# Happy-ZZX/PL-VIWO

Hardware: AMD Instinct MI355X
Metric: frames/sec (track+EKF update), 752x480 mono, 250 pts+80 lines; ATE vs CPU ref (higher is better)
Workload: dtype f64

## Files before the change

### pl-viwo_amd/csrc/camera_tracks.hpp

```cpp
#pragma once
#include <algorithm>
#include <cstdint>
#include <unordered_map>
#include <utility>
#include <vector>

#include "../../include/plviwo.h"

namespace plv {

inline int bounding_start_host(const plv_state_view &st, double t) {
  const int N = st.n_clones;
  if (N < 4) return -1;
  const double *ct = st.clone_time;
  if (t < ct[0] - st.dt_exp || t > ct[N - 1] + st.dt_exp) return -1;
  if (t > ct[N - 1]) return -1;
  int n_b = -1;
  for (int i = 0; i < N - 1; ++i)
    if (ct[i] - st.dt_exp <= t && t <= ct[i + 1] + st.dt_exp) {
      n_b = i;
      break;
    }
  if (n_b < 0) return -1;
  int start = n_b - 1;
  if (n_b - 1 < 0)
    start = 0;
  else if (n_b + 2 >= N)
    start = N - 4;
  if (start < 0 || start + 4 > N) return -1;
  return start;
}
inline bool has_bounding_poses(const plv_state_view &st, double t) { return bounding_start_host(st, t) >= 0; }

struct BoundingMemo {
  const plv_state_view &st;
  double t[40];
  int s0[40];
  int n = 0;
  explicit BoundingMemo(const plv_state_view &s) : st(s) {}
  int operator()(double tq) {
    for (int i = n - 1; i >= 0; --i)
      if (t[i] == tq) return s0[i];
    const int r = bounding_start_host(st, tq);
    if (n < 40) t[n] = tq, s0[n++] = r;
    return r;
  }
};

struct Track {
  static constexpr int W = 2;
  static constexpr int P = 3;
  std::vector<double> t;
  std::vector<float> uv, uvn;
  int li = -1;
  unsigned long long li_seq = 0;
};

struct LineTrack {
  static constexpr int W = 4;
  static constexpr int P = 6;
  std::vector<double> t;
  std::vector<float> uv, uvn;
  std::vector<int> points;
  int D = 0;
};

inline void copy_track_meta(Track &, const Track &) {}
inline void copy_track_meta(LineTrack &dst, const LineTrack &src) {
  if (dst.t.empty() && dst.points.empty()) {
    dst.D = src.D;
    dst.points = src.points;
  }
}

template <class TrackT> struct PoolCand {
  uint64_t id;
  TrackT tr;
};
template <class TrackT> using TrackMap = std::unordered_map<uint64_t, TrackT>;

template <class TrackT> void append_obs(TrackT &dst, const TrackT &src, size_t i) {
  constexpr size_t W = TrackT::W;
  dst.t.push_back(src.t[i]);
  dst.uv.insert(dst.uv.end(), src.uv.begin() + W * i, src.uv.begin() + W * (i + 1));
  dst.uvn.insert(dst.uvn.end(), src.uvn.begin() + W * i, src.uvn.begin() + W * (i + 1));
}

template <class TrackT> void give_back(TrackMap<TrackT> &unused, uint64_t id, const TrackT &src, size_t i) {
  TrackT &u = unused[id];
  copy_track_meta(u, src);
  append_obs(u, src, i);
}

template <class TrackT> void give_back_all(TrackMap<TrackT> &unused, PoolCand<TrackT> &c) {
  if (unused.find(c.id) == unused.end()) {
    unused.emplace(c.id, std::move(c.tr));
    c.tr = TrackT{};
    return;
  }
  for (size_t i = 0; i < c.tr.t.size(); ++i) give_back(unused, c.id, c.tr, i);
}

template <class TrackT, class Keep> size_t trim_track(TrackT &tr, Keep keep) {
  constexpr size_t W = TrackT::W;
  size_t n = 0;
  for (size_t i = 0; i < tr.t.size(); ++i) {
    if (!keep(i)) continue;
    if (n != i) {
      tr.t[n] = tr.t[i];
      std::copy(tr.uv.begin() + W * i, tr.uv.begin() + W * (i + 1), tr.uv.begin() + W * n);
      std::copy(tr.uvn.begin() + W * i, tr.uvn.begin() + W * (i + 1), tr.uvn.begin() + W * n);
    }
    ++n;
  }
  tr.t.resize(n);
  tr.uv.resize(W * n);
  tr.uvn.resize(W * n);
  return n;
}

template <class TrackT> size_t drop_before(TrackT &tr, double t) {
  return trim_track(tr, [&tr, t](size_t i) { return !(tr.t[i] < t); });
}

template <class TrackT> size_t trim_to_window(TrackMap<TrackT> &unused, uint64_t id, TrackT &tr, double dt, double t_new, double t_old) {
  return trim_track(tr, [&unused, id, &tr, dt, t_new, t_old](size_t i) {
    const double tm = tr.t[i] + dt;
    if (tm > t_new) {
      give_back(unused, id, tr, i);
      return false;
    }
    return !(tm < t_old);
  });
}

template <class TrackT> void take_pool(TrackMap<TrackT> &db, double t_old, double t_new, std::vector<PoolCand<TrackT>> &pool) {
  static thread_local std::vector<std::pair<uint64_t, typename TrackMap<TrackT>::iterator>> take;
  take.clear();
  for (auto it = db.begin(); it != db.end(); ++it) {
    bool older = false, newer = false;
    for (double t : it->second.t) {
      older = older || t < t_old;
      newer = newer || t > t_new;
    }
    if (older || !newer) take.emplace_back(it->first, it);
  }
  std::sort(take.begin(), take.end(), [](const auto &a, const auto &b) { return a.first < b.first; });
  pool.reserve(pool.size() + take.size());
  for (auto &tk : take) pool.push_back(PoolCand<TrackT>{tk.first, std::move(db.extract(tk.second).mapped())});
}

template <class TrackT> void sort_long_first(std::vector<PoolCand<TrackT>> &pool) {
  static thread_local std::vector<std::pair<int, int>> ord;
  ord.clear();
  for (size_t i = 0; i < pool.size(); ++i) ord.emplace_back(-(int)pool[i].tr.t.size(), (int)i);
  std::sort(ord.begin(), ord.end());
  std::vector<PoolCand<TrackT>> sorted;
  sorted.reserve(pool.size());
  for (const auto &o : ord) sorted.push_back(std::move(pool[(size_t)o.second]));
  pool.swap(sorted);
}

template <class TrackT>
void flatten_pool(const std::vector<PoolCand<TrackT>> &pool, std::vector<int> &ptr, std::vector<double> &t, std::vector<float> &uv, std::vector<float> &uvn) {
  constexpr size_t W = TrackT::W;
  ptr.assign(pool.size() + 1, 0);
  for (size_t f = 0; f < pool.size(); ++f) ptr[f + 1] = ptr[f] + (int)pool[f].tr.t.size();
  const size_t nobs = (size_t)ptr.back();
  t.resize(nobs), uv.resize(W * nobs), uvn.resize(W * nobs);
  for (size_t f = 0; f < pool.size(); ++f) {
    const TrackT &tr = pool[f].tr;
    std::copy(tr.t.begin(), tr.t.end(), t.begin() + ptr[f]);
    std::copy(tr.uv.begin(), tr.uv.end(), uv.begin() + W * ptr[f]);
    std::copy(tr.uvn.begin(), tr.uvn.end(), uvn.begin() + W * ptr[f]);
  }
}

struct CpiPoses {
  bool on = false, noise = false;
  std::vector<double> R, p, Q;
  std::vector<int> C;
};

template <class TrackT>
int cpi_attach(plv_ctx *ctx, const plv_state_view *st, const plv_cpi_table *cpi, bool noise, double dt, std::vector<PoolCand<TrackT>> &pool,
               TrackMap<TrackT> &unused, CpiPoses &out) {
  std::vector<double> tq;
  for (const PoolCand<TrackT> &c : pool)
    for (double t : c.tr.t) tq.push_back(t + dt);
  std::vector<double> Rq(9 * tq.size()), pq(3 * tq.size());
  std::vector<uint8_t> okq(tq.size());
// ... 94 lines not shown
      if (seen++ < S.n_skip[f] || fused_ran) continue;
      gather_obs(S.g, c.tr, i, cpi, ptr[f] + i);
    }
    S.sptr[q + 1] = (int)S.g.t.size();
    std::copy(feat_all + P * f, feat_all + P * (f + 1), S.feat.begin() + P * q);
    if (ids_out) ids_out[q] = c.id;
  }
}

template <class TrackT, class StartOf, class Whole>
int return_rejected(const std::vector<PoolCand<TrackT>> &pool, const Selection<TrackT> &S, double dt, StartOf &start_of, TrackMap<TrackT> &unused,
                    uint8_t *accepted_out, Whole whole) {
  int n_accepted = 0;
  for (size_t q = 0; q < S.sel.size(); ++q) {
    n_accepted += S.acc[q];
    if (accepted_out) accepted_out[q] = S.acc[q];
    if (S.acc[q] || whole(S.sel[q])) continue;
    const PoolCand<TrackT> &c = pool[S.sel[q]];
    for (size_t i = 0; i < c.tr.t.size(); ++i)
      if (start_of(c.tr.t[i] + dt) >= 0) give_back(unused, c.id, c.tr, i);
  }
  return n_accepted;
}

template <class TrackT> typename TrackMap<TrackT>::iterator put_track(TrackMap<TrackT> &db, uint64_t id, TrackT &tr) {
  auto ins = db.try_emplace(id);
  TrackT &d = ins.first->second;
  if (ins.second) {
    d = std::move(tr);
  } else {
    d.t.insert(d.t.end(), tr.t.begin(), tr.t.end());
    d.uv.insert(d.uv.end(), tr.uv.begin(), tr.uv.end());
    d.uvn.insert(d.uvn.end(), tr.uvn.begin(), tr.uvn.end());
  }
  return ins.first;
}

}
```

### pl-viwo_amd/csrc/jacobian_kernels.hip

```cpp
#include <hip/hip_runtime.h>
namespace plv {
#define JAC_NSTAMP 32
__device__ long long *g_jac_stamps = nullptr;
__device__ __forceinline__ void jac_stamp(int id) {
  long long *s = g_jac_stamps;
  if (s && threadIdx.x == 0) s[blockIdx.x * JAC_NSTAMP + id] = (long long)__builtin_amdgcn_s_memtime();
}
}
#define GATE_STAMP(id) jac_stamp(id)
#include "cam_models.hpp"
#include "gate_core.hpp"
#include "jacobian_kernels.hpp"
#include "nullspace_core.hpp"
#include "so3.hpp"

namespace plv {

__device__ int bounding_start(const JacParams &P, double t) {
  const int N = P.n_clones;
  if (N < 4) return -1;
  const double *ct = P.clone_time;
  if (t < ct[0] - P.dt_exp || t > ct[N - 1] + P.dt_exp) return -1;
  if (t > ct[N - 1]) return -1;
  int n_b = -1;
  for (int i = 0; i < N - 1; ++i)
    if (ct[i] - P.dt_exp <= t && t <= ct[i + 1] + P.dt_exp) {
      n_b = i;
      break;
    }
  if (n_b < 0) return -1;
  int start = n_b - 1;
  if (n_b - 1 < 0)
    start = 0;
  else if (n_b + 2 >= N)
    start = N - 4;
  if (start < 0 || start + 4 > N) return -1;
  return start;
}

struct Interp {
  M3 R;
  V3 p;
  M3 Ho[4];
  double lam[4];
  double dtj[6];
};
// ... 40 lines not shown
  const M3 Jl = Jl_so3(A_ori);
  M3 H0o = Rio;
  double lsum = 0;
#pragma unroll
  for (int w = 0; w < 3; ++w) {
    const M3 JinvW = inv3(Jl_so3(th[w]));
    H0o = ma(H0o, ms(mm(Jl, mm(JinvW, Rw[w])), -lam[w]));
    o.Ho[w + 1] = ms(mm(Jl, JinvW), lam[w]);
    o.lam[w + 1] = lam[w];
    lsum += lam[w];
  }
  o.Ho[0] = H0o;
  o.lam[0] = 1.0 - lsum;
  V3 dori{{0, 0, 0}}, dpos{{0, 0, 0}};
#pragma unroll
  for (int w = 0; w < 3; ++w) {
    dori = vadd(dori, vsc(th[w], lamd[w]));
    dpos = vadd(dpos, vsc(dp[w], lamd[w]));
  }
  const V3 top = vsc(mv(Jl, dori), -1.0);
#pragma unroll
  for (int i = 0; i < 3; ++i) {
    o.dtj[i] = top[i];
    o.dtj[3 + i] = dpos[i];
  }
}


struct WinTab {
  M3 R0, Rw[3], JinvW[3], Vi;
  V3 p0, th[3], dp[3];
  double vrow[3][3];
};
#define JAC_MAX_WIN 40

__device__ __forceinline__ void build_window_tables(const JacParams &P, WinTab *tab, const double *Rt = nullptr, const double *pt = nullptr) {
  const int nwin = max(P.n_clones - 3, 0);
  const int ntask = nwin * (Rt ? 3 : 2);
  const double *const R_est = P.clone_R, *const R_fej = P.clone_R_fej, *const p_est = P.clone_p, *const p_fej = P.clone_p_fej;
  for (int idx = threadIdx.x; idx < ntask * 3; idx += blockDim.x) {
    const int w = idx % 3, e = idx / 3;
    const bool second = e >= 2 * nwin;
    const int s0 = second ? e - 2 * nwin : e >> 1, fej = second ? 0 : e & 1;
    const double *Rs = second ? Rt : (fej ? R_fej : R_est), *ps = second ? pt : (fej ? p_fej : p_est);
    WinTab &T = tab[e];
    const M3 R0 = ldM(Rs + 9 * s0);
    const V3 p0 = ldV(ps + 3 * s0);
    const M3 Rw = mm(ldM(Rs + 9 * (s0 + 1 + w)), tp(R0));
    const V3 th = log_so3(Rw);
    T.Rw[w] = Rw;
    T.th[w] = th;
    T.dp[w] = vsub(ldV(ps + 3 * (s0 + 1 + w)), p0);
    const double d = P.clone_time[s0 + 1 + w] - P.clone_time[s0];
    T.vrow[w][0] = d;
    T.vrow[w][1] = d * d;
    T.vrow[w][2] = d * d * d;
    if (fej) T.JinvW[w] = inv3(Jl_so3(th));
    if (w == 0) {
      T.R0 = R0;
      T.p0 = p0;
    }
  }
  __syncthreads();
  for (int e = threadIdx.x; e < ntask; e += blockDim.x) {
    M3 V;
#pragma unroll
    for (int w = 0; w < 3; ++w)
// ... 1996 lines not shown
```

### pl-viwo_amd/csrc/line_api.hip

```cpp
#include <algorithm>
#include <chrono>
#include <cmath>
#include <cstring>
#include <atomic>
#include <condition_variable>
#include <functional>
#include <memory>
#include <map>
#include <mutex>
#include <thread>
#include <unordered_map>
#include <vector>

#include "line_host.hpp"
#include "cam_models.hpp"
#include "line_kernels.hpp"
#include "update_state.hpp"
#include "plv_internal.hpp"
#include "camera_tracks.hpp"
#include "update_tail.hpp"

using namespace plv;
using namespace plv::linehost;

// ... 37 lines not shown
  std::vector<float> uv, uvn;
  std::vector<uint8_t> has, flags;
  CpiPoses cpi;
  std::vector<double> lg_two_step;
  std::vector<uint8_t> ok_two_step;
  double us_pool = 0;
  plv_line_tracks view() const {
    plv_line_tracks all{};
    all.n_lines = Lp, all.obs_ptr = ptr.data(), all.obs_time = ot.data(), all.seg_uv = uv.data(), all.seg_uvn = uvn.data();
    all.D = D.data(), all.anchor_pt = anchor.data(), all.has_pt = has.data();
    if (cpi.on) all.res_R = cpi.R.data(), all.res_p = cpi.p.data();
    return all;
  }
};

struct LineTracker {
  LinePool pool_prep;
  LinesJob ujob;
  std::vector<float> lines_last;
  std::vector<uint64_t> ids_last;
  std::vector<int> rel_ptr_last{0};
  std::vector<uint64_t> rel_id_last;
  uint64_t currid = 1;
  bool walk_on_device = false;
  int walk_mode = 0;
  struct WalkInfo {
    int mode = 0, n_components = 0, longest_component = 0, n_chains = 0, fell_back = 0;
  } winfo;
  bool chains_valid = false;
  std::vector<FldChain> last_chains;
  int last_pts_extent = 0;
  DevBuf comps, recs, recs_sorted;
  bool prefetch = false;
  std::unordered_map<uint64_t, LineTrack> db;
  DevBuf half, map, work, pts, chains, counts, segs, seg_count, uv_in, uv_out;
  DevBuf lab, lab_cnt, lab_roots;
  hipStream_t ccl_stream = nullptr;
  hipEvent_t canny_done = nullptr, labels_ready = nullptr;
  PinBuf pin;
  hipEvent_t edges_ready = nullptr;
  std::vector<uint64_t> dec_ids;
  std::vector<double> dec_vals;
  const uint8_t *early_raw = nullptr;
  const unsigned *early_hist = nullptr;
  int early_w = 0, early_h = 0;
  int pending_which = -1, pending_fed = -1;
  bool defer_finish = false;
  std::function<void()> deferred;
  std::atomic<int> defer_state{0};
  struct TriState {
    bool valid = false;
    plv_state_view view;
    std::vector<double> clone_time, clone_R, clone_p;
    std::vector<int> clone_id;
  } tri_state;
  std::vector<float> cached;
  int cached_which = -1, cached_fed = -1;
  std::mutex mtx;
  linehost::Job job;
  std::thread worker;
  std::mutex jm;
  std::condition_variable jcv;
  std::atomic<int> job_state{0};
  struct FeedJob {
    plv_ctx *ctx = nullptr;
    double timestamp = 0, vps[6] = {0, 0, 0, 0, 0, 0};
    double K8[8] = {0, 0, 0, 0, 0, 0, 0, 0};
// ... 577 lines not shown
  auto F0 = std::chrono::steady_clock::now();
  const int nl = (int)lines.size() / 4;
  plv::counters().lines_detected += (unsigned long long)nl;
  std::vector<uint64_t> ids(nl);
  for (int i = 0; i < nl; ++i) ids[i] = ++T->currid;
  Assign A;
  assign_points_parallel(&T->host, fit_threads().load(std::memory_order_relaxed), lines.data(), nl, pts, pids, np, A);
  auto F1 = std::chrono::steady_clock::now();
  const int nk = (int)A.kept.size();
  std::vector<float> fl(4 * (size_t)nk);
  std::vector<uint64_t> fid(nk);
  for (int q = 0; q < nk; ++q) {
    std::copy(lines.begin() + 4 * A.kept[q], lines.begin() + 4 * A.kept[q] + 4, fl.begin() + 4 * q);
    fid[q] = ids[A.kept[q]];
  }
  const bool first = T->lines_last.empty();
  auto F_match = F1, F_und = F1;
  if (!first) {
    std::vector<int> match((size_t)std::max(nk, 1));
    match_lines_parallel(&T->host, fit_threads().load(std::memory_order_relaxed), fl.data(), nk, A.rel_ptr.data(), A.rel_id.data(), T->lines_last.data(),
                         (int)T->ids_last.size(), T->rel_ptr_last.data(), T->rel_id_last.data(), match.data());
    for (int q = 0; q < nk; ++q)
      if (match[q] >= 0) fid[q] = (uint64_t)(int)T->ids_last[match[q]];
    if (timing) F_match = std::chrono::steady_clock::now();
    std::vector<float> un(4 * (size_t)std::max(nk, 1));
    for (int q = 0; q < 2 * nk; ++q)
      undistort_model(cam_model, K8, fl[2 * (size_t)q], fl[2 * (size_t)q + 1], un[2 * (size_t)q], un[2 * (size_t)q + 1]);
    if (timing) F_und = std::chrono::steady_clock::now();
    for (int q = 0; q < nk; ++q) {
      const int D = plv_line_classification(fl.data() + 4 * q, vps);
      auto ins = T->db.try_emplace(fid[q]);
      const bool is_new = ins.second;
      LineTrack &tr = ins.first->second;
      if (is_new) {
        tr.D = D;
        tr.t.reserve(32);
        tr.uv.reserve(128);
        tr.uvn.reserve(128);
      }
      tr.t.push_back(timestamp);
      tr.uv.insert(tr.uv.end(), fl.begin() + 4 * q, fl.begin() + 4 * q + 4);
      tr.uvn.insert(tr.uvn.end(), un.begin() + 4 * q, un.begin() + 4 * q + 4);
      for (int p = A.rel_ptr[q]; p < A.rel_ptr[q + 1]; ++p) tr.points.push_back((int)A.rel_id[p]);
    }
  }
  T->lines_last.swap(fl);
  T->ids_last.swap(fid);
  T->rel_ptr_last = A.rel_ptr;
  T->rel_id_last = A.rel_id;
  if (timing) {
    auto us = [](auto a, auto b) { return std::chrono::duration<double, std::micro>(b - a).count(); };
    fprintf(stderr, "line feed: kept-line copy + match %.1f us, undistort %.1f us, classify + store -> end %.1f us\n", us(F1, F_match), us(F_match, F_und),
            us(F_und, std::chrono::steady_clock::now()));
    fprintf(stderr, "line feed: assignment %.1f us (%d lines x %d points), match + undistort + classify + store %.1f us (%d kept)\n", us(F0, F1), nl, np,
            us(F1, std::chrono::steady_clock::now()), nk);
  }
  return PLV_OK;
}

}
namespace plv {
int plv_line_tracker_feed_async_points(plv_ctx *ctx, double timestamp, const double *vps, int np, const float *pts, const uint64_t *pids) {
  if (!ctx || !vps || np < 0 || (np > 0 && (!pts || !pids))) return PLV_E_BADARG;
  LineTracker *T = ltr(ctx);
  std::lock_guard<std::mutex> lk(T->mtx);
  LineTracker::FeedJob &F = T->feed;
  F.pts.assign(pts, pts + 2 * (size_t)np);
  F.pids.assign(pids, pids + (size_t)np);
  const bool detecting = !T->walk_on_device && T->worker.joinable() && T->pending_which == PLV_PYR_CUR && T->pending_fed == plv_front_fed_count(ctx);
  if (!detecting) {
    F.pool_on = false;
    F.rc = feed_points_impl(ctx, T, timestamp, vps, np, F.pts.data(), F.pids.data(), ctx->cfg.intrinsics, ctx->cam_model);
    return F.rc;
  }
  g_feed_impl = feed_points_impl;
// ... 80 lines not shown
      if (seg_uvn) std::copy(tr.uvn.begin(), tr.uvn.end(), seg_uvn + 4 * (size_t)no);
      no += m;
      if (D) D[i] = tr.D;
      if (pts_ptr) {
        if (npt + (int)tr.points.size() > pts_cap) return PLV_E_CAPACITY;
        if (pt_ids) std::copy(tr.points.begin(), tr.points.end(), pt_ids + npt);
        npt += (int)tr.points.size();
      }
    } else if (D) {
      D[i] = 0;
    }
    obs_ptr[i + 1] = no;
    if (pts_ptr) pts_ptr[i + 1] = npt;
  }
  return PLV_OK;
}

int plv_line_db_remove(plv_ctx *ctx, const uint64_t *ids, int n_ids) {
  if (!ctx || (n_ids > 0 && !ids)) return PLV_E_BADARG;
  LineTracker *T = ltr(ctx);
  std::lock_guard<std::mutex> lk(T->mtx);
  for (int i = 0; i < n_ids; ++i) T->db.erase(ids[i]);
  return PLV_OK;
}

int plv_line_db_append_measurements(plv_ctx *ctx, uint64_t id, int n, const double *t, const float *seg_uv,
                                    const float *seg_uvn, int D, const int *point_ids, int n_pts) {
  if (!ctx || n < 0 || (n > 0 && (!t || !seg_uv || !seg_uvn)) || (n_pts > 0 && !point_ids)) return PLV_E_BADARG;
  LineTracker *T = ltr(ctx);
  std::lock_guard<std::mutex> lk(T->mtx);
  const bool is_new = T->db.find(id) == T->db.end();
  LineTrack &tr = T->db[id];
  if (is_new) tr.D = D;
  tr.t.insert(tr.t.end(), t, t + n);
  tr.uv.insert(tr.uv.end(), seg_uv, seg_uv + 4 * (size_t)n);
  tr.uvn.insert(tr.uvn.end(), seg_uvn, seg_uvn + 4 * (size_t)n);
  tr.points.insert(tr.points.end(), point_ids, point_ids + n_pts);
  return PLV_OK;
}

}
namespace plv {
void plv_line_defer_finish(plv_ctx *ctx, int on) { ltr(ctx, false)->defer_finish = on != 0; }
void plv_line_run_deferred(plv_ctx *ctx) { (void)ltr(ctx); }
}
extern "C" {

namespace {
struct LineWaitHook {
  plv_ctx *ctx;
  std::function<void()> *fn;
};
void line_wait_hook(void *arg) {
  LineWaitHook *h = (LineWaitHook *)arg;
  plv_tracker_run_deferred(h->ctx);
  if (h->fn && *h->fn) (*h->fn)();
}
}

namespace {
void form_line_pool(LineTracker *T, const PoolArgs &A, LinePool &R) {
  R = LinePool();
  R.valid = true;
  R.t_prev_frame = A.t_prev_frame, R.state_time = A.state_time, R.dt = A.dt, R.n_clones = A.n_clones;
  R.t_oldest = A.t_oldest, R.t_oldest2 = A.t_oldest2;
  const double dt = R.dt, t_oldest = R.t_oldest, t_oldest2 = R.t_oldest2;
  const PoolArgs *opt = &A;
  plv::HostPhase ph_scan("line pool: scan + take");
  {
    std::lock_guard<std::mutex> lk(T->mtx);
    R.db_size_before = (int)T->db.size();
    take_pool(T->db, t_oldest2 - dt, opt->t_prev_frame - dt, R.pool);
  }
  ph_scan.stop();
  plv::HostPhase ph_trim("line pool: trim + sort");
  R.n_pool = (int)R.pool.size();
  R.unused.reserve(R.pool.size());
  size_t kept_cands = 0;
  for (size_t ci = 0; ci < R.pool.size(); ++ci) {
    PoolCand<LineTrack> &c = R.pool[ci];
    if (trim_to_window(R.unused, c.id, c.tr, dt, opt->state_time + 0.01, t_oldest - 0.01) >= 2) {
      if (kept_cands != ci) R.pool[kept_cands] = std::move(c);
      ++kept_cands;
    }
  }
  R.pool.resize(kept_cands);
  sort_long_first(R.pool);
}
}

namespace {
void discard_line_pool(LineTracker *T) {
  LinePool &R = T->pool_prep;
  if (!R.valid) return;
  std::lock_guard<std::mutex> lk(T->mtx);
  auto put = [&](uint64_t id, LineTrack &tr) {
    const bool is_new = T->db.find(id) == T->db.end();
    LineTrack &d = T->db[id];
    if (is_new) {
      d = std::move(tr);
      return;
    }
    const size_t na = d.t.size(), nb = tr.t.size();
    std::vector<std::pair<double, std::pair<int, int>>> order;
    order.reserve(na + nb);
    for (size_t i = 0; i < na; ++i) order.push_back({d.t[i], {0, (int)i}});
    for (size_t i = 0; i < nb; ++i) order.push_back({tr.t[i], {1, (int)i}});
    std::stable_sort(order.begin(), order.end(), [](const auto &a, const auto &b) { return a.first < b.first; });
    LineTrack m;
    copy_track_meta(m, d);
    for (const auto &e : order) append_obs(m, e.second.first ? tr : d, (size_t)e.second.second);
    d = std::move(m);
  };
  for (auto &c : R.pool) put(c.id, c.tr);
  for (auto &kv : R.unused) put(kv.first, kv.second);
  R = LinePool();
}
}

}
namespace plv {
int plv_line_pool_prepare(plv_ctx *ctx, const plv_state_view *st, const plv_update_options *opt) {
  if (!ctx || !st || !opt || opt->cpi || st->n_clones < 2 || st->dt_state_id >= 0) return 1;
  LineTracker *T;
  {
    std::lock_guard<std::mutex> lk(g_mtx);
    auto it = g_lt.find(ctx);
    if (it == g_lt.end()) return 1;
    T = it->second;
  }
  {
    std::lock_guard<std::mutex> lk(T->jm);
    if (T->feed_state == 1) return 0;
  }
  T = ltr(ctx);
  if (T->feed.rc != PLV_OK) return 1;
  const PoolArgs A = PoolArgs::of(st, opt);
  const LinePool &R = T->pool_prep;
  if (R.valid && R.t_prev_frame == A.t_prev_frame && R.state_time == A.state_time && R.dt == A.dt && R.n_clones == A.n_clones && R.t_oldest == A.t_oldest &&
      R.t_oldest2 == A.t_oldest2)
    return 1;
  plv::HostPhase ph("update_lines: pool formed inside the point update's wait");
  discard_line_pool(T);
  form_line_pool(T, A, T->pool_prep);
  return 1;
// ... 369 lines not shown
```

### pl-viwo_amd/csrc/tracker_api.hip

```cpp
#include <algorithm>
#include <cmath>
#include <functional>
#include <memory>
#include <mutex>
#include <unordered_map>
#include <vector>

#include <sys/resource.h>
#include "plv_ctx.hpp"
#include "update_state.hpp"
#include "plv_internal.hpp"
#include "gate_stage.hpp"
#include "camera_tracks.hpp"
#include "update_tail.hpp"

using plv::Track;

namespace {

struct Tracker {
  std::vector<float> pts_last;
  std::vector<uint64_t> ids_last;
  std::vector<uint8_t> mask_last;
  uint64_t currid = 0;
  int detect_ahead = 2;
  bool ahead_deferred = false;
  bool defer_db = false;
  const plv_state_view *early_st = nullptr;
  const plv_update_options *early_lines = nullptr;
  int early_cap = 0;
  std::unordered_map<uint64_t, int> chain_index;
  bool chain_ok = false;
  std::function<void()> deferred_db;
  std::unordered_map<uint64_t, Track> db;
  struct UsedPoint {
    double p[3], newest;
  };
  std::unordered_map<uint64_t, UsedPoint> used;
  struct Listed {
    uint64_t id;
    Track tr;
    double p[3];
  };
  std::vector<Listed> last_slam, last_init;
  std::vector<uint64_t> dec_ids;
  std::vector<double> dec_vals;
  const plv_state_view *spec_st = nullptr;
  const plv_update_options *spec_opt = nullptr;
  std::function<void(int, const float *, const uint64_t *)> points_ready;
  unsigned long long feed_seq = 0;
  std::vector<double> frame_t;
  struct Spec {
    bool active = false;
    double t_prev_frame = 0, state_time = 0, dt = 0, t_oldest = 0, t_oldest2 = 0;
    int n_clones = 0, max_msckf = 0, max_obs = 0, k = 0, F = 0;
    std::unordered_map<uint64_t, int> index;
    std::vector<uint64_t> ids;
    std::vector<int> ptr, li, cols;
    std::vector<uint8_t> meta, prevalid, flags;
    std::vector<double> ot;
    std::vector<float> ouv, ouvn;
  } spec;
  std::mutex mtx;
};

std::mutex g_mtx;
std::unordered_map<plv_ctx *, Tracker *> g_trk;
// ... 284 lines not shown
    keep_mask();
    return PLV_OK;
  }
  n = (int)T->ids_last.size();
  std::copy(T->pts_last.begin(), T->pts_last.end(), pts.begin());
  std::copy(T->ids_last.begin(), T->ids_last.end(), ids.begin());
  {
    plv::HostPhase ph("tracker_feed: perform_detection");
    TRY(plv_perform_detection(ctx, PLV_PYR_LAST, T->mask_last.empty() ? nullptr : T->mask_last.data(), pts.data(), ids.data(), n,
                              cap, &T->currid, &n));
  }
  std::vector<float> pts_new(pts.begin(), pts.begin() + 2 * (size_t)n), n1(2 * (size_t)std::max(n, 1));
  std::vector<uint8_t> mask_ll((size_t)std::max(n, 1), 0);
  std::vector<Track *> tp;
  if (n == 0) {
    launch_prefetch();
    T->pts_last.clear();
    T->ids_last.clear();
    keep_mask();
    return PLV_OK;
  }
  {
    plv::HostPhase ph("tracker_feed: perform_matching");
    launch_prefetch();
    const int rc_l = plv_perform_matching_launch(ctx, n, pts.data(), pts_new.data());
    if (rc_l == PLV_OK) plv_line_run_deferred(ctx);
    TRY(rc_l);
    tp.assign((size_t)n, nullptr);
    for (int i = 0; i < n; ++i) {
      auto it = T->db.find(ids[i]);
      if (it == T->db.end()) continue;
      Track &tr = it->second;
      tp[i] = &tr;
      if (!tr.t.empty()) {
        __builtin_prefetch(&tr.t.back() + 1, 1);
        __builtin_prefetch(&tr.uv.back() + 1, 1);
        __builtin_prefetch(&tr.uvn.back() + 1, 1);
      }
    }
    if (T->spec_st && T->spec_opt && !mask) spec_submit(ctx, T, timestamp, n, ids.data(), tp.data());
    plv::NsScope ns_wait(plv::counters().flow_wait_ns);
    TRY(plv_perform_matching_wait(ctx, pts_new.data(), mask_ll.data(), nullptr, n1.data(), nullptr));
  }
  plv::HostPhase ph_db("tracker_feed: database update");
  std::vector<float> good;
  std::vector<uint64_t> good_ids;
  std::vector<uint8_t> is_good((size_t)n, 0);
  good.reserve(2 * (size_t)n), good_ids.reserve((size_t)n);
  for (int i = 0; i < n; ++i) {
    const float x = pts_new[2 * i], y = pts_new[2 * i + 1];
    if (x < 0 || y < 0 || (int)x >= W || (int)y >= H) continue;
    if (mask && mask[(size_t)(int)y * W + (int)x] > 127) continue;
    if (!mask_ll[i]) continue;
    is_good[i] = 1;
    good.push_back(x);
    good.push_back(y);
    good_ids.push_back(ids[i]);
  }
  if (T->points_ready) T->points_ready((int)good_ids.size(), good.data(), good_ids.data());
  for (int i = 0; i < n; ++i) {
    if (!is_good[i]) continue;
    const float x = pts_new[2 * i], y = pts_new[2 * i + 1];
    Track &tr = tp[i] ? *tp[i] : T->db[ids[i]];
    if (tr.t.capacity() == 0) {
      tr.t.reserve(32);
      tr.uv.reserve(64);
      tr.uvn.reserve(64);
    }
    tr.t.push_back(timestamp);
    tr.uv.push_back(x);
    tr.uv.push_back(y);
    tr.uvn.push_back(n1[2 * i]);
    tr.uvn.push_back(n1[2 * i + 1]);
  }
  T->pts_last.swap(good);
  T->ids_last.swap(good_ids);
  keep_mask();
  T->ahead_deferred = T->detect_ahead == 2 && !T->ids_last.empty();
  if (T->detect_ahead == 1 && !T->ids_last.empty())
    (void)plv_perform_detection_ahead(ctx, mask, T->pts_last.data(), T->ids_last.data(), (int)T->ids_last.size());
  return PLV_OK;
}

static void start_detection_ahead(void *arg) {
  plv_ctx *ctx = (plv_ctx *)arg;
  Tracker *T = trk(ctx);
  {
    std::lock_guard<std::mutex> lk(T->mtx);
    if (T->ahead_deferred) {
      T->ahead_deferred = false;
      (void)plv_perform_detection_ahead(ctx, T->mask_last.empty() ? nullptr : T->mask_last.data(), T->pts_last.data(), T->ids_last.data(),
                                        (int)T->ids_last.size());
    }
  }
}
static int poll_line_pool(void *arg) {
  plv_ctx *ctx = (plv_ctx *)arg;
  Tracker *T = trk(ctx);
  if (!T->early_lines || !T->early_st) return 1;
  if (!plv_line_pool_prepare(ctx, T->early_st, T->early_lines)) return 0;
  if (plv::host_phases().on) {
    plv::host_phases().add("chain: pool ready inside the point wait (count)", 1.0);
    if (!T->chain_ok) plv::host_phases().add("chain: no - the point pool exceeds max_msckf or holds no candidate (count)", 1.0);
    if (!ctx->chain.ready) plv::host_phases().add("chain: no - state variables not chainable (count)", 1.0);
    if (!plv_update_state(ctx)->applied_armed) plv::host_phases().add("chain: no - the point launch did not arm the applied word (count)", 1.0);
  }
// ... 86 lines not shown
      for (int i = 0; i < m; ++i) {
        if (obs_time) obs_time[at + i] = tr.t[i];
        if (obs_uv) obs_uv[2 * (at + i)] = tr.uv[2 * i], obs_uv[2 * (at + i) + 1] = tr.uv[2 * i + 1];
        if (obs_uvn) obs_uvn[2 * (at + i)] = tr.uvn[2 * i], obs_uvn[2 * (at + i) + 1] = tr.uvn[2 * i + 1];
      }
      at += m;
    }
    obs_ptr[f + 1] = at;
  }
  return PLV_OK;
}

int plv_db_cleanup_measurements(plv_ctx *ctx, double t) {
  if (!ctx) return PLV_E_BADARG;
  Tracker *T = trk(ctx);
  std::lock_guard<std::mutex> lk(T->mtx);
  for (auto it = T->db.begin(); it != T->db.end();) it = drop_before(it->second, t) == 0 ? T->db.erase(it) : std::next(it);
  return PLV_OK;
}

int plv_db_remove(plv_ctx *ctx, const uint64_t *ids, int n) {
  if (!ctx || (n > 0 && !ids)) return PLV_E_BADARG;
  Tracker *T = trk(ctx);
  std::lock_guard<std::mutex> lk(T->mtx);
  for (int i = 0; i < n; ++i) T->db.erase(ids[i]);
  return PLV_OK;
}

int plv_db_append_measurements(plv_ctx *ctx, uint64_t id, int n, const double *t, const float *uv, const float *uvn) {
  if (!ctx || n < 0 || (n > 0 && (!t || !uv || !uvn))) return PLV_E_BADARG;
  Tracker *T = trk(ctx);
  std::lock_guard<std::mutex> lk(T->mtx);
  Track &tr = T->db[id];
  tr.t.insert(tr.t.end(), t, t + n);
  tr.uv.insert(tr.uv.end(), uv, uv + 2 * (size_t)n);
  tr.uvn.insert(tr.uvn.end(), uvn, uvn + 2 * (size_t)n);
  return PLV_OK;
}

int plv_db_disparity(plv_ctx *ctx, double time0, double time1, double *mean, double *std, int *n) {
  if (!ctx || !mean || !std || !n) return PLV_E_BADARG;
  Tracker *T = trk(ctx);
  std::lock_guard<std::mutex> lk(T->mtx);
  std::vector<std::pair<uint64_t, double>> disp;
  for (auto &kv : T->db) {
    const Track &tr = kv.second;
    const auto it0 = std::find(tr.t.begin(), tr.t.end(), time0), it1 = std::find(tr.t.begin(), tr.t.end(), time1);
    if (it0 == tr.t.end() || it1 == tr.t.end()) continue;
    const size_t i0 = it0 - tr.t.begin(), i1 = it1 - tr.t.begin();
    const float du = tr.uv[2 * i1] - tr.uv[2 * i0], dv = tr.uv[2 * i1 + 1] - tr.uv[2 * i0 + 1];
    disp.emplace_back(kv.first, (double)std::sqrt(du * du + dv * dv));
  }
  if (disp.size() < 2) {
    *mean = -1.0, *std = -1.0, *n = 0;
    return PLV_OK;
  }
  std::sort(disp.begin(), disp.end());
  double m = 0.0, var = 0.0;
  for (auto &d : disp) m += d.second;
  m /= (double)disp.size();
  for (auto &d : disp) var += (d.second - m) * (d.second - m);
  *mean = m;
  *std = std::sqrt(var / (double)(disp.size() - 1));
  *n = (int)disp.size();
  return PLV_OK;
}

namespace {
typedef PoolCand<Track> Cand;
// ... 40 lines not shown
  }
  int finish_early(bool updated) {
    if (!updated) std::fill(dx, dx + ctx->cov_n, 0.0);
    return finish(PLV_OK);
  }
  int abandon(int rc) {
    for (Cand &c : pool) give_back_all(unused, c);
    return finish(rc);
  }

  void slam_landmarks() {
    std::lock_guard<std::mutex> lk(T->mtx);
    for (int i = 0; i < opt->n_slam; ++i) {
      auto it = T->db.find(opt->slam_ids[i]);
      if (it == T->db.end()) continue;
      Track &tr = it->second;
      const size_t keep = trim_to_window(unused, it->first, tr, dt, opt->state_time + st->dt_exp, t_oldest - st->dt_exp);
      if (keep == 0) continue;
      Tracker::Listed e{it->first, Track{}, {0, 0, 0}};
      for (size_t q = 0; q < keep; ++q)
        if (start_of(tr.t[q] + dt) >= 0) append_obs(e.tr, tr, q);
      if (!e.tr.t.empty()) T->last_slam.push_back(std::move(e));
    }
  }

  bool is_slam(uint64_t id) const { return std::find(opt->slam_ids, opt->slam_ids + opt->n_slam, id) != opt->slam_ids + opt->n_slam; }

  void take_pool_of_window() {
    {
      std::lock_guard<std::mutex> lk(T->mtx);
      take_pool(T->db, t_oldest2 - dt, opt->t_prev_frame - dt, pool);
    }
    res->n_pool = (int)pool.size();
    size_t kept_cands = 0;
    for (size_t ci = 0; ci < pool.size(); ++ci) {
      Cand &c = pool[ci];
      const size_t keep = trim_to_window(unused, c.id, c.tr, dt, opt->state_time + st->dt_exp, t_oldest - st->dt_exp);
      if (keep == 1 && is_slam(c.id)) give_back(unused, c.id, c.tr, 0);
      if (keep < 2) continue;
      if (kept_cands != ci) pool[kept_cands] = std::move(c);
      ++kept_cands;
    }
    pool.resize(kept_cands);
    sort_long_first(pool);
  }

  int collect_speculative() {
    Tracker::Spec &S = T->spec;
    S.active = false;
    const int Fp0 = (int)pool.size();
    const bool same = S.t_prev_frame == opt->t_prev_frame && S.state_time == opt->state_time && S.dt == dt && S.n_clones == st->n_clones &&
                      S.t_oldest == t_oldest && S.t_oldest2 == t_oldest2 && S.max_msckf == opt->max_msckf && S.max_obs == opt->max_obs && !opt->cpi &&
                      opt->max_slam == 0 && opt->n_slam == 0;
    std::vector<int> cand_of(Fp0, -1);
    bool known = true;
    for (int f = 0; f < Fp0; ++f) {
      const auto it = S.index.find(pool[f].id);
      if (it == S.index.end()) known = false;
      else cand_of[f] = it->second;
    }
    T->chain_index.clear();
    T->chain_ok = same && known && Fp0 <= plv::spec_grid(opt->max_msckf);
    if (T->chain_ok && T->early_lines)
      for (int f = 0; f < Fp0; ++f)
        if (usable_views(pool[f].tr, dt, start_of) >= 2) T->chain_index.emplace(pool[f].id, cand_of[f]);
    std::vector<double> cp(3 * (size_t)S.F), ce(S.F);
    std::vector<uint8_t> cok(S.F), cacc(S.F), cmem(S.F);
    int count = 0, over = 0, nrows = 0;
    int rc_s;
    {
      plv::RoctxRange rx_upd("[Time-Cam] MSCKF update");
      plv::HostPhase ph_dev("update_points: device submission + wait");
      rc_s = plv_points_update_collect(ctx, cp.data(), cok.data(), ce.data(), cacc.data(), &nrows, dx, start_detection_ahead, ctx, cmem.data(), &count, &over);
    }
    T->chain_ok = false;
    auto fail = [&](const char *why) {
      plv::set_last_error("speculative point update: %s (host pool %d, device pool %d%s)", why, Fp0, count, over ? ", over the cap" : "");
// ... 491 lines not shown
```

Baseline: 2216.

## Store track observations inline with cached time bounds and slab-allocated maps

Track storage moves from std::vector to a small-buffer InlineVec sized to hold a full sliding window, so per-track observations no longer need heap allocations. Each track also caches its min and max timestamps, which lets take_pool, drop_before and trim_to_window skip the per-observation scans when nothing falls outside the window. The track hash maps switch to a slab allocator for their nodes, and the pool compaction is folded into sort_long_first through a keep mask. In exchange, track objects get much larger, so moving them copies inline buffers instead of swapping pointers, and the cached bounds must stay consistent on every mutation path.

Result: no change. 2242, median of 3 (+1.2%).

```diff
diff --git a/pl-viwo_amd/csrc/camera_tracks.hpp b/pl-viwo_amd/csrc/camera_tracks.hpp
--- a/pl-viwo_amd/csrc/camera_tracks.hpp
+++ b/pl-viwo_amd/csrc/camera_tracks.hpp
@@ -1,11 +1,15 @@
 #pragma once
 #include <algorithm>
 #include <cstdint>
+#include <functional>
+#include <limits>
 #include <unordered_map>
 #include <utility>
 #include <vector>
 
 #include "../../include/plviwo.h"
+#include "inline_vec.hpp"
+#include "track_limits.hpp"
 
 namespace plv {
 
@@ -47,21 +51,44 @@
   }
 };
 
-struct Track {
+struct TrackTimes {
+  double t_min = std::numeric_limits<double>::infinity(), t_max = -std::numeric_limits<double>::infinity();
+  TrackTimes() = default;
+  TrackTimes(const TrackTimes &) = default;
+  TrackTimes &operator=(const TrackTimes &) = default;
+  TrackTimes(TrackTimes &&o) noexcept : t_min(o.t_min), t_max(o.t_max) { o.reset_times(); }
+  TrackTimes &operator=(TrackTimes &&o) noexcept {
+    const double lo = o.t_min, hi = o.t_max;
+    o.reset_times();
+    t_min = lo, t_max = hi;
+    return *this;
+  }
+  void reset_times() { t_min = std::numeric_limits<double>::infinity(), t_max = -std::numeric_limits<double>::infinity(); }
+  void note_time(double t) {
+    if (t < t_min) t_min = t;
+    if (t > t_max) t_max = t;
+  }
+  void note_times(const TrackTimes &o) {
+    if (o.t_min < t_min) t_min = o.t_min;
+    if (o.t_max > t_max) t_max = o.t_max;
+  }
+};
+
+struct Track : TrackTimes {
   static constexpr int W = 2;
   static constexpr int P = 3;
-  std::vector<double> t;
-  std::vector<float> uv, uvn;
+  InlineVec<double, TRACK_INLINE_OBS> t;
+  InlineVec<float, W * TRACK_INLINE_OBS> uv, uvn;
   int li = -1;
   unsigned long long li_seq = 0;
 };
 
-struct LineTrack {
+struct LineTrack : TrackTimes {
   static constexpr int W = 4;
   static constexpr int P = 6;
-  std::vector<double> t;
-  std::vector<float> uv, uvn;
-  std::vector<int> points;
+  InlineVec<double, TRACK_INLINE_OBS> t;
+  InlineVec<float, W * TRACK_INLINE_OBS> uv, uvn;
+  InlineVec<int, LINE_POINTS_PER_OBS * TRACK_INLINE_OBS> points;
   int D = 0;
 };
 
@@ -77,11 +104,22 @@
   uint64_t id;
   TrackT tr;
 };
-template <class TrackT> using TrackMap = std::unordered_map<uint64_t, TrackT>;
+template <class TrackT>
+using TrackMap = std::unordered_map<uint64_t, TrackT, std::hash<uint64_t>, std::equal_to<uint64_t>,
+                                    SlabAlloc<std::pair<const uint64_t, TrackT>, sizeof(std::pair<const uint64_t, TrackT>)>>;
+
+template <class TrackT> void append_raw(TrackT &tr, double t, const float *uv, const float *uvn) {
+  constexpr size_t W = TrackT::W;
+  tr.t.push_back(t);
+  tr.note_time(t);
+  tr.uv.insert(tr.uv.end(), uv, uv + W);
+  tr.uvn.insert(tr.uvn.end(), uvn, uvn + W);
+}
 
 template <class TrackT> void append_obs(TrackT &dst, const TrackT &src, size_t i) {
   constexpr size_t W = TrackT::W;
   dst.t.push_back(src.t[i]);
+  dst.note_time(src.t[i]);
   dst.uv.insert(dst.uv.end(), src.uv.begin() + W * i, src.uv.begin() + W * (i + 1));
   dst.uvn.insert(dst.uvn.end(), src.uvn.begin() + W * i, src.uvn.begin() + W * (i + 1));
 }
@@ -104,8 +142,10 @@
 template <class TrackT, class Keep> size_t trim_track(TrackT &tr, Keep keep) {
   constexpr size_t W = TrackT::W;
   size_t n = 0;
+  TrackTimes kept;
   for (size_t i = 0; i < tr.t.size(); ++i) {
     if (!keep(i)) continue;
+    kept.note_time(tr.t[i]);
     if (n != i) {
       tr.t[n] = tr.t[i];
       std::copy(tr.uv.begin() + W * i, tr.uv.begin() + W * (i + 1), tr.uv.begin() + W * n);
@@ -116,14 +156,17 @@
   tr.t.resize(n);
   tr.uv.resize(W * n);
   tr.uvn.resize(W * n);
+  tr.t_min = kept.t_min, tr.t_max = kept.t_max;
   return n;
 }
 
 template <class TrackT> size_t drop_before(TrackT &tr, double t) {
+  if (!(tr.t_min < t)) return tr.t.size();
   return trim_track(tr, [&tr, t](size_t i) { return !(tr.t[i] < t); });
 }
 
 template <class TrackT> size_t trim_to_window(TrackMap<TrackT> &unused, uint64_t id, TrackT &tr, double dt, double t_new, double t_old) {
+  if (!(tr.t_max + dt > t_new) && !(tr.t_min + dt < t_old)) return tr.t.size();
   return trim_track(tr, [&unused, id, &tr, dt, t_new, t_old](size_t i) {
     const double tm = tr.t[i] + dt;
     if (tm > t_new) {
@@ -137,26 +180,25 @@
 template <class TrackT> void take_pool(TrackMap<TrackT> &db, double t_old, double t_new, std::vector<PoolCand<TrackT>> &pool) {
   static thread_local std::vector<std::pair<uint64_t, typename TrackMap<TrackT>::iterator>> take;
   take.clear();
-  for (auto it = db.begin(); it != db.end(); ++it) {
-    bool older = false, newer = false;
-    for (double t : it->second.t) {
-      older = older || t < t_old;
-      newer = newer || t > t_new;
-    }
-    if (older || !newer) take.emplace_back(it->first, it);
-  }
+  for (auto it = db.begin(); it != db.end(); ++it)
+    if (it->second.t_min < t_old || !(it->second.t_max > t_new)) take.emplace_back(it->first, it);
   std::sort(take.begin(), take.end(), [](const auto &a, const auto &b) { return a.first < b.first; });
   pool.reserve(pool.size() + take.size());
-  for (auto &tk : take) pool.push_back(PoolCand<TrackT>{tk.first, std::move(db.extract(tk.second).mapped())});
-}
-
-template <class TrackT> void sort_long_first(std::vector<PoolCand<TrackT>> &pool) {
+  for (auto &tk : take) {
+    pool.emplace_back();
+    pool.back().id = tk.first;
+    pool.back().tr = std::move(db.extract(tk.second).mapped());
+  }
+}
+
+template <class TrackT> void sort_long_first(std::vector<PoolCand<TrackT>> &pool, const std::vector<uint8_t> *keep = nullptr) {
   static thread_local std::vector<std::pair<int, int>> ord;
   ord.clear();
-  for (size_t i = 0; i < pool.size(); ++i) ord.emplace_back(-(int)pool[i].tr.t.size(), (int)i);
+  for (size_t i = 0; i < pool.size(); ++i)
+    if (!keep || (*keep)[i]) ord.emplace_back(-(int)pool[i].tr.t.size(), (int)i);
   std::sort(ord.begin(), ord.end());
   std::vector<PoolCand<TrackT>> sorted;
-  sorted.reserve(pool.size());
+  sorted.reserve(ord.size());
   for (const auto &o : ord) sorted.push_back(std::move(pool[(size_t)o.second]));
   pool.swap(sorted);
 }
@@ -317,8 +359,22 @@
     d.t.insert(d.t.end(), tr.t.begin(), tr.t.end());
     d.uv.insert(d.uv.end(), tr.uv.begin(), tr.uv.end());
     d.uvn.insert(d.uvn.end(), tr.uvn.begin(), tr.uvn.end());
+    d.note_times(tr);
   }
   return ins.first;
 }
 
-}
+template <class TrackT> void merge_by_time(TrackT &d, const TrackT &tr) {
+  const size_t na = d.t.size(), nb = tr.t.size();
+  std::vector<std::pair<double, std::pair<int, int>>> order;
+  order.reserve(na + nb);
+  for (size_t i = 0; i < na; ++i) order.push_back({d.t[i], {0, (int)i}});
+  for (size_t i = 0; i < nb; ++i) order.push_back({tr.t[i], {1, (int)i}});
+  std::stable_sort(order.begin(), order.end(), [](const auto &a, const auto &b) { return a.first < b.first; });
+  TrackT m;
+  copy_track_meta(m, d);
+  for (const auto &e : order) append_obs(m, e.second.first ? tr : d, (size_t)e.second.second);
+  d = std::move(m);
+}
+
+}
diff --git a/pl-viwo_amd/csrc/inline_vec.hpp b/pl-viwo_amd/csrc/inline_vec.hpp
--- /dev/null
+++ b/pl-viwo_amd/csrc/inline_vec.hpp
@@ -0,0 +1,215 @@
+#pragma once
+#include <algorithm>
+#include <atomic>
+#include <cstddef>
+#include <cstdint>
+#include <cstring>
+#include <initializer_list>
+#include <new>
+#include <type_traits>
+#include <utility>
+#include <vector>
+
+namespace plv {
+
+template <class T, size_t N> class InlineVec {
+  static_assert(std::is_trivially_copyable<T>::value && std::is_trivially_destructible<T>::value, "InlineVec holds plain values");
+  static_assert(N > 0, "InlineVec needs an inline capacity");
+  T *heap_ = nullptr;
+  uint32_t size_ = 0, cap_ = (uint32_t)N;
+  alignas(T) unsigned char buf_[N * sizeof(T)];
+
+  T *inl() { return reinterpret_cast<T *>(buf_); }
+  const T *inl() const { return reinterpret_cast<const T *>(buf_); }
+  void grow_to(size_t cap) {
+    T *p = static_cast<T *>(::operator new(cap * sizeof(T)));
+    if (size_) std::memcpy(p, data(), size_ * sizeof(T));
+    if (heap_) ::operator delete(heap_);
+    heap_ = p, cap_ = (uint32_t)cap;
+  }
+  void room_for(size_t n) {
+    if (n > cap_) grow_to(std::max(n, 2 * (size_t)cap_));
+  }
+  void unspill() {
+    if (!heap_) return;
+    if (size_) std::memcpy(buf_, heap_, size_ * sizeof(T));
+    ::operator delete(heap_);
+    heap_ = nullptr, cap_ = (uint32_t)N;
+  }
+  void take(InlineVec &o) {
+    if (o.heap_) {
+      heap_ = o.heap_, cap_ = o.cap_;
+      o.heap_ = nullptr, o.cap_ = (uint32_t)N;
+    } else if (o.size_) {
+      std::memcpy(buf_, o.buf_, o.size_ * sizeof(T));
+    }
+    size_ = o.size_, o.size_ = 0;
+  }
+
+ public:
+  typedef T value_type;
+  typedef T *iterator;
+  typedef const T *const_iterator;
+  static constexpr size_t inline_capacity = N;
+
+  InlineVec() {}
+  InlineVec(const InlineVec &o) { assign(o.begin(), o.end()); }
+  InlineVec(InlineVec &&o) noexcept { take(o); }
+  InlineVec(std::initializer_list<T> il) { assign(il.begin(), il.end()); }
+  InlineVec &operator=(std::initializer_list<T> il) {
+    assign(il.begin(), il.end());
+    return *this;
+  }
+  InlineVec &operator=(const InlineVec &o) {
+    if (this != &o) assign(o.begin(), o.end());
+    return *this;
+  }
+  InlineVec &operator=(InlineVec &&o) noexcept {
+    if (this == &o) return *this;
+    if (heap_) ::operator delete(heap_);
+    heap_ = nullptr, cap_ = (uint32_t)N;
+    take(o);
+    return *this;
+  }
+  ~InlineVec() {
+    if (heap_) ::operator delete(heap_);
+  }
+
+  size_t size() const { return size_; }
+  bool empty() const { return size_ == 0; }
+  size_t capacity() const { return cap_; }
+  bool spilled() const { return heap_ != nullptr; }
+  T *data() { return heap_ ? heap_ : inl(); }
+  const T *data() const { return heap_ ? heap_ : inl(); }
+  T *begin() { return data(); }
+  const T *begin() const { return data(); }
+  T *end() { return data() + size_; }
+  const T *end() const { return data() + size_; }
+  T &operator[](size_t i) { return data()[i]; }
+  const T &operator[](size_t i) const { return data()[i]; }
+  T &front() { return data()[0]; }
+  const T &front() const { return data()[0]; }
+  T &back() { return data()[size_ - 1]; }
+  const T &back() const { return data()[size_ - 1]; }
+
+  void reserve(size_t n) { room_for(n); }
+  void clear() {
+    size_ = 0;
+    unspill();
+  }
+  void resize(size_t n) {
+    if (n > size_) {
+      room_for(n);
+      std::memset(static_cast<void *>(data() + size_), 0, (n - size_) * sizeof(T));
+    }
+    size_ = (uint32_t)n;
+    if (n <= N) unspill();
+  }
+  void push_back(const T &v) {
+    const T x = v;
+    room_for((size_t)size_ + 1);
+    data()[size_++] = x;
+  }
+  void pop_back() { --size_; }
+  template <class It> void assign(It first, It last) {
+    size_ = 0;
+    const size_t n = (size_t)(last - first);
+    if (n <= N) unspill();
+    room_for(n);
+    T *d = data();
+    for (size_t i = 0; i < n; ++i, ++first) d[i] = *first;
+    size_ = (uint32_t)n;
+  }
+  template <class It> void insert(const_iterator pos, It first, It last) {
+    (void)pos;
+    const size_t n = (size_t)(last - first);
+    room_for(size_ + n);
+    T *d = data() + size_;
+    for (size_t i = 0; i < n; ++i, ++first) d[i] = *first;
+    size_ += (uint32_t)n;
+  }
+};
+
+struct SlabArena {
+  static constexpr size_t slab_bytes = 32768;
+  size_t block = 0, per_slab = 0;
+  static size_t rounded(size_t bytes) { return (bytes + 63) & ~(size_t)63; }
+  void *free_list = nullptr;
+  std::vector<void *> slabs;
+  std::atomic<size_t> refs{1};
+  size_t live = 0;
+  void *get(size_t bytes) {
+    if (!block) block = rounded(bytes), per_slab = std::max<size_t>(8, slab_bytes / block);
+    if (!free_list) {
+      char *s = static_cast<char *>(::operator new(block * per_slab, std::align_val_t(64)));
+      slabs.push_back(s);
+      for (size_t i = per_slab; i-- > 0;) {
+        void *b = s + i * block;
+        *static_cast<void **>(b) = free_list;
+        free_list = b;
+      }
+    }
+    void *b = free_list;
+    free_list = *static_cast<void **>(b);
+    ++live;
+    return b;
+  }
+  void put(void *b) {
+    *static_cast<void **>(b) = free_list;
+    free_list = b;
+    --live;
+  }
+  ~SlabArena() {
+    for (void *s : slabs) ::operator delete(s, std::align_val_t(64));
+  }
+};
+
+template <class U, size_t MinNode> class SlabAlloc {
+  template <class, size_t> friend class SlabAlloc;
+  SlabArena *a_;
+  static constexpr bool is_node = sizeof(U) >= MinNode && sizeof(U) >= sizeof(void *) && alignof(U) <= 64;
+  bool from_arena(size_t n) const { return is_node && n == 1 && (a_->block == 0 || a_->block == SlabArena::rounded(sizeof(U))); }
+
+ public:
+  typedef U value_type;
+  typedef std::true_type propagate_on_container_move_assignment;
+  typedef std::true_type propagate_on_container_copy_assignment;
+  typedef std::true_type propagate_on_container_swap;
+  typedef std::false_type is_always_equal;
+  template <class V> struct rebind {
+    typedef SlabAlloc<V, MinNode> other;
+  };
+
+  SlabAlloc() : a_(new SlabArena()) {}
+  SlabAlloc(const SlabAlloc &o) noexcept : a_(o.a_) { a_->refs.fetch_add(1, std::memory_order_relaxed); }
+  template <class V> SlabAlloc(const SlabAlloc<V, MinNode> &o) noexcept : a_(o.a_) { a_->refs.fetch_add(1, std::memory_order_relaxed); }
+  SlabAlloc &operator=(const SlabAlloc &o) noexcept {
+    o.a_->refs.fetch_add(1, std::memory_order_relaxed);
+    release();
+    a_ = o.a_;
+    return *this;
+  }
+  ~SlabAlloc() { release(); }
+  SlabAlloc select_on_container_copy_construction() const { return SlabAlloc(); }
+
+  U *allocate(size_t n) {
+    if (from_arena(n)) return static_cast<U *>(a_->get(sizeof(U)));
+    return static_cast<U *>(::operator new(n * sizeof(U)));
+  }
+  void deallocate(U *p, size_t n) noexcept {
+    if (from_arena(n) && a_->block)
+      a_->put(p);
+    else
+      ::operator delete(p);
+  }
+  template <class V> bool operator==(const SlabAlloc<V, MinNode> &o) const { return a_ == o.a_; }
+  template <class V> bool operator!=(const SlabAlloc<V, MinNode> &o) const { return a_ != o.a_; }
+  const SlabArena &arena() const { return *a_; }
+
+ private:
+  void release() {
+    if (a_->refs.fetch_sub(1, std::memory_order_acq_rel) == 1) delete a_;
+  }
+};
+
+}
diff --git a/pl-viwo_amd/csrc/jacobian_kernels.hip b/pl-viwo_amd/csrc/jacobian_kernels.hip
--- a/pl-viwo_amd/csrc/jacobian_kernels.hip
+++ b/pl-viwo_amd/csrc/jacobian_kernels.hip
@@ -12,6 +12,7 @@
 #include "gate_core.hpp"
 #include "jacobian_kernels.hpp"
 #include "nullspace_core.hpp"
+#include "track_limits.hpp"
 #include "so3.hpp"
 
 namespace plv {
@@ -118,7 +119,6 @@
   V3 p0, th[3], dp[3];
   double vrow[3][3];
 };
-#define JAC_MAX_WIN 40
 
 __device__ __forceinline__ void build_window_tables(const JacParams &P, WinTab *tab, const double *Rt = nullptr, const double *pt = nullptr) {
   const int nwin = max(P.n_clones - 3, 0);
diff --git a/pl-viwo_amd/csrc/line_api.hip b/pl-viwo_amd/csrc/line_api.hip
--- a/pl-viwo_amd/csrc/line_api.hip
+++ b/pl-viwo_amd/csrc/line_api.hip
@@ -93,7 +93,7 @@
   int last_pts_extent = 0;
   DevBuf comps, recs, recs_sorted;
   bool prefetch = false;
-  std::unordered_map<uint64_t, LineTrack> db;
+  TrackMap<LineTrack> db;
   DevBuf half, map, work, pts, chains, counts, segs, seg_count, uv_in, uv_out;
   DevBuf lab, lab_cnt, lab_roots;
   hipStream_t ccl_stream = nullptr;
@@ -737,15 +737,8 @@
       auto ins = T->db.try_emplace(fid[q]);
       const bool is_new = ins.second;
       LineTrack &tr = ins.first->second;
-      if (is_new) {
-        tr.D = D;
-        tr.t.reserve(32);
-        tr.uv.reserve(128);
-        tr.uvn.reserve(128);
-      }
-      tr.t.push_back(timestamp);
-      tr.uv.insert(tr.uv.end(), fl.begin() + 4 * q, fl.begin() + 4 * q + 4);
-      tr.uvn.insert(tr.uvn.end(), un.begin() + 4 * q, un.begin() + 4 * q + 4);
+      if (is_new) tr.D = D;
+      append_raw(tr, timestamp, &fl[4 * (size_t)q], &un[4 * (size_t)q]);
       for (int p = A.rel_ptr[q]; p < A.rel_ptr[q + 1]; ++p) tr.points.push_back((int)A.rel_id[p]);
     }
   }
@@ -892,9 +885,7 @@
   const bool is_new = T->db.find(id) == T->db.end();
   LineTrack &tr = T->db[id];
   if (is_new) tr.D = D;
-  tr.t.insert(tr.t.end(), t, t + n);
-  tr.uv.insert(tr.uv.end(), seg_uv, seg_uv + 4 * (size_t)n);
-  tr.uvn.insert(tr.uvn.end(), seg_uvn, seg_uvn + 4 * (size_t)n);
+  for (int i = 0; i < n; ++i) append_raw(tr, t[i], seg_uv + 4 * (size_t)i, seg_uvn + 4 * (size_t)i);
   tr.points.insert(tr.points.end(), point_ids, point_ids + n_pts);
   return PLV_OK;
 }
@@ -936,16 +927,13 @@
   plv::HostPhase ph_trim("line pool: trim + sort");
   R.n_pool = (int)R.pool.size();
   R.unused.reserve(R.pool.size());
-  size_t kept_cands = 0;
+  static thread_local std::vector<uint8_t> stays;
+  stays.assign(R.pool.size(), 0);
   for (size_t ci = 0; ci < R.pool.size(); ++ci) {
     PoolCand<LineTrack> &c = R.pool[ci];
-    if (trim_to_window(R.unused, c.id, c.tr, dt, opt->state_time + 0.01, t_oldest - 0.01) >= 2) {
-      if (kept_cands != ci) R.pool[kept_cands] = std::move(c);
-      ++kept_cands;
-    }
-  }
-  R.pool.resize(kept_cands);
-  sort_long_first(R.pool);
+    stays[ci] = trim_to_window(R.unused, c.id, c.tr, dt, opt->state_time + 0.01, t_oldest - 0.01) >= 2;
+  }
+  sort_long_first(R.pool, &stays);
 }
 }
 
@@ -961,16 +949,7 @@
       d = std::move(tr);
       return;
     }
-    const size_t na = d.t.size(), nb = tr.t.size();
-    std::vector<std::pair<double, std::pair<int, int>>> order;
-    order.reserve(na + nb);
-    for (size_t i = 0; i < na; ++i) order.push_back({d.t[i], {0, (int)i}});
-    for (size_t i = 0; i < nb; ++i) order.push_back({tr.t[i], {1, (int)i}});
-    std::stable_sort(order.begin(), order.end(), [](const auto &a, const auto &b) { return a.first < b.first; });
-    LineTrack m;
-    copy_track_meta(m, d);
-    for (const auto &e : order) append_obs(m, e.second.first ? tr : d, (size_t)e.second.second);
-    d = std::move(m);
+    merge_by_time(d, tr);
   };
   for (auto &c : R.pool) put(c.id, c.tr);
   for (auto &kv : R.unused) put(kv.first, kv.second);
diff --git a/pl-viwo_amd/csrc/track_limits.hpp b/pl-viwo_amd/csrc/track_limits.hpp
--- /dev/null
+++ b/pl-viwo_amd/csrc/track_limits.hpp
@@ -0,0 +1,13 @@
+#pragma once
+
+#define JAC_MAX_WIN 40
+
+namespace plv {
+constexpr int TRACK_MAX_CLONES = JAC_MAX_WIN / 2 + 3;
+constexpr int TRACK_MAX_OBS = 24;
+constexpr int TRACK_INLINE_OBS = (TRACK_MAX_CLONES > TRACK_MAX_OBS ? TRACK_MAX_CLONES : TRACK_MAX_OBS) + 1 + 3;
+static_assert(TRACK_INLINE_OBS >= JAC_MAX_WIN / 2 + 3 + 1, "a full window plus the frame's observation stays inline");
+static_assert(TRACK_INLINE_OBS >= TRACK_MAX_OBS + 1, "max_obs observations plus the frame's own stay inline");
+static_assert(TRACK_INLINE_OBS >= 20 + 1 + 3, "the shipped 20-clone window stays inline with room to spare");
+constexpr int LINE_POINTS_PER_OBS = 4;
+}
diff --git a/pl-viwo_amd/csrc/tracker_api.hip b/pl-viwo_amd/csrc/tracker_api.hip
--- a/pl-viwo_amd/csrc/tracker_api.hip
+++ b/pl-viwo_amd/csrc/tracker_api.hip
@@ -32,7 +32,7 @@
   std::unordered_map<uint64_t, int> chain_index;
   bool chain_ok = false;
   std::function<void()> deferred_db;
-  std::unordered_map<uint64_t, Track> db;
+  plv::TrackMap<Track> db;
   struct UsedPoint {
     double p[3], newest;
   };
@@ -383,11 +383,6 @@
       if (it == T->db.end()) continue;
       Track &tr = it->second;
       tp[i] = &tr;
-      if (!tr.t.empty()) {
-        __builtin_prefetch(&tr.t.back() + 1, 1);
-        __builtin_prefetch(&tr.uv.back() + 1, 1);
-        __builtin_prefetch(&tr.uvn.back() + 1, 1);
-      }
     }
     if (T->spec_st && T->spec_opt && !mask) spec_submit(ctx, T, timestamp, n, ids.data(), tp.data());
     plv::NsScope ns_wait(plv::counters().flow_wait_ns);
@@ -413,16 +408,8 @@
     if (!is_good[i]) continue;
     const float x = pts_new[2 * i], y = pts_new[2 * i + 1];
     Track &tr = tp[i] ? *tp[i] : T->db[ids[i]];
-    if (tr.t.capacity() == 0) {
-      tr.t.reserve(32);
-      tr.uv.reserve(64);
-      tr.uvn.reserve(64);
-    }
-    tr.t.push_back(timestamp);
-    tr.uv.push_back(x);
-    tr.uv.push_back(y);
-    tr.uvn.push_back(n1[2 * i]);
-    tr.uvn.push_back(n1[2 * i + 1]);
+    const float xy[2] = {x, y};
+    append_raw(tr, timestamp, xy, &n1[2 * i]);
   }
   T->pts_last.swap(good);
   T->ids_last.swap(good_ids);
@@ -575,9 +562,7 @@
   Tracker *T = trk(ctx);
   std::lock_guard<std::mutex> lk(T->mtx);
   Track &tr = T->db[id];
-  tr.t.insert(tr.t.end(), t, t + n);
-  tr.uv.insert(tr.uv.end(), uv, uv + 2 * (size_t)n);
-  tr.uvn.insert(tr.uvn.end(), uvn, uvn + 2 * (size_t)n);
+  for (int i = 0; i < n; ++i) append_raw(tr, t[i], uv + 2 * (size_t)i, uvn + 2 * (size_t)i);
   return PLV_OK;
 }
 
@@ -684,17 +669,14 @@
       take_pool(T->db, t_oldest2 - dt, opt->t_prev_frame - dt, pool);
     }
     res->n_pool = (int)pool.size();
-    size_t kept_cands = 0;
+    std::vector<uint8_t> stays(pool.size(), 0);
     for (size_t ci = 0; ci < pool.size(); ++ci) {
       Cand &c = pool[ci];
       const size_t keep = trim_to_window(unused, c.id, c.tr, dt, opt->state_time + st->dt_exp, t_oldest - st->dt_exp);
       if (keep == 1 && is_slam(c.id)) give_back(unused, c.id, c.tr, 0);
-      if (keep < 2) continue;
-      if (kept_cands != ci) pool[kept_cands] = std::move(c);
-      ++kept_cands;
-    }
-    pool.resize(kept_cands);
-    sort_long_first(pool);
+      stays[ci] = keep >= 2;
+    }
+    sort_long_first(pool, &stays);
   }
 
   int collect_speculative() {
```
